# tylerlum/Vine_Robot_IsaacGymEnvs

Measured on AMD Instinct MI355X. Metric: env-steps/sec Vine5LinkMovingBase 16384 envs per GPU, higher is better.
Workload: dtype f32 (env step, rollout inference); update: fp16 GEMM operands and backward-only saved activations (gates, saved cell states, dG, dh), f32 accumulate / recurrent state / heads / loss / optimiser, device-side GradScaler loss scaling (mixed_precision: True = the reference YAML's value, PY:53); rollout

## Files before the change

### vine_robot_isaacgymenvs_amd/csrc/ppo_kernels.hip

```cpp

#include <hip/hip_runtime.h>

#include <cstdio>
#include <cstdlib>

#include "../../include/vine.h"
#include "../../include/vine_ppo.h"
#include "vine_policy_head.h"
#include "vine_ppo_formulas.h"

namespace {

__device__ __forceinline__ float4 ld4(const float* p) { return *reinterpret_cast<const float4*>(p); }
__device__ __forceinline__ void st4(float* p, float4 v) { *reinterpret_cast<float4*>(p) = v; }

typedef unsigned short lp16_t;
typedef __attribute__((__vector_size__(2 * sizeof(float)))) float f32x2_hw;
#ifdef VINE_LP_BF16
typedef __bf16 lp16_hw;
#define VINE_LP16_NAME "bf16"
#define MFMA_LP16_BUILTIN __builtin_amdgcn_mfma_f32_16x16x32_bf16
#define DS_READ_TR16_B64 __builtin_amdgcn_ds_read_tr16_b64_v4bf16
typedef __bf16 lp16_tr_hw;
#define LP16_MAX 3.3895314e38f
#else
typedef _Float16 lp16_hw;
#define VINE_LP16_NAME "fp16"
#define MFMA_LP16_BUILTIN __builtin_amdgcn_mfma_f32_16x16x32_f16
#define DS_READ_TR16_B64 __builtin_amdgcn_ds_read_tr16_b64_v4f16
typedef __fp16 lp16_tr_hw;
#define LP16_MAX 65504.0f
#endif
typedef __attribute__((__vector_size__(2 * sizeof(lp16_hw)))) lp16_hw lp16x2_hw;
__device__ __forceinline__ lp16_t f2lp(float f) {
    const lp16_hw h = (lp16_hw)f;
    return *reinterpret_cast<const lp16_t*>(&h);
}
__device__ __forceinline__ unsigned f2lp2(float lo, float hi) {
    const f32x2_hw v = {lo, hi};
    const lp16x2_hw h = __builtin_convertvector(v, lp16x2_hw);
    return *reinterpret_cast<const unsigned*>(&h);
}
#ifdef VINE_LP_BF16
__device__ __forceinline__ float lp2f(lp16_t h) { return __uint_as_float((unsigned)h << 16); }
__device__ __forceinline__ void unpack2(unsigned r, float& lo, float& hi) {
    lo = __uint_as_float(r << 16);
    hi = __uint_as_float(r & 0xFFFF0000u);
}
#else
__device__ __forceinline__ float lp2f(lp16_t h) { return (float)*reinterpret_cast<const lp16_hw*>(&h); }
__device__ __forceinline__ void unpack2(unsigned r, float& lo, float& hi) {
    const lp16x2_hw h = *reinterpret_cast<const lp16x2_hw*>(&r);
    lo = (float)h[0];
    hi = (float)h[1];
}
#endif
__device__ __forceinline__ float4 ld4(const lp16_t* p) {
    const uint2 r = *reinterpret_cast<const uint2*>(p);
    float4 v;
    unpack2(r.x, v.x, v.y);
    unpack2(r.y, v.z, v.w);
    return v;
}
__device__ __forceinline__ void st4(lp16_t* p, float4 v) {
    uint2 r;
    r.x = f2lp2(v.x, v.y);
    r.y = f2lp2(v.z, v.w);
    *reinterpret_cast<uint2*>(p) = r;
}

template <typename HP>
__global__ void lstm_fwd_kernel(long long B, int H, const float* __restrict__ igates, long long ig_stride,
                                const float* __restrict__ hgates, const float* __restrict__ bias,
                                const float* __restrict__ c_prev, const unsigned char* __restrict__ done,
                                long long done_stride, float* __restrict__ h_out, long long h_stride,
                                float* __restrict__ c_out, HP* __restrict__ gates_act,
                                HP* __restrict__ hp_next, const unsigned char* __restrict__ done_next,
                                long long done_next_stride, long long hp_stride) {
    const int H4 = H >> 2;
    const long long total = B * H4;
    for (long long idx = (long long)blockIdx.x * blockDim.x + threadIdx.x; idx < total;
         idx += (long long)gridDim.x * blockDim.x) {
        const long long b = idx / H4;
        const int j = (int)(idx - b * H4) << 2;
        const float keep = done ? 1.0f - (float)done[b * done_stride] : 1.0f;
        const float* ig = igates + b * ig_stride;
        float4 g[4];
// ... 2060 lines not shown
#pragma unroll
            for (int c = 0; c < 8; ++c)
#pragma unroll
                for (int e = 0; e < 4; ++e) wbits |= (((q[c] >> (8 * e)) & 0xffu) ? 1u : 0u) << (4 * c + e);
            dwords[it] = wbits;
        }
    }
#define WGW_LOAD(S, it)                                                                                        \
    {                                                                                                          \
        const long long t_ = (it) < stages ? (it) : stages - 1;           \
        ra_##S = *reinterpret_cast<const uint4*>(asrc + t_ * 32 * ldy);                                        \
        rb0_##S = *reinterpret_cast<const uint4*>(bsrc0 + t_ * bstep0);                                        \
        rb1_##S = *reinterpret_cast<const uint4*>(bsrc1 + t_ * bstep1);                                        \
        rb2_##S = *reinterpret_cast<const uint4*>(bsrc2 + t_ * bstep2);                                        \
        __builtin_amdgcn_sched_barrier(0);             \
    }
     \
#define WGW_MASKED(v, bit)                                                                                     \
    ([&] { const unsigned m_ = (dw_##bit) ? 0u : 0xffffffffu; return make_uint4((v).x & m_, (v).y & m_, (v).z & m_, (v).w & m_); }())
#define WGW_STORE(S, buf, it)                                                                                  \
    {                                                                                                          \
        const unsigned dw_ = SEQ ? dwords[(it) < stages ? (it) : stages - 1] : 0u;                             \
        const unsigned dw_dbit0 = dw_ & dbit0, dw_dbit1 = dw_ & dbit1, dw_dbit2 = dw_ & dbit2;                 \
        if (aval) *reinterpret_cast<uint4*>(&al[buf][aoff]) = ra_##S;                                          \
        *reinterpret_cast<uint4*>(&bl[buf][boff0]) = WGW_MASKED(rb0_##S, dbit0);                               \
        *reinterpret_cast<uint4*>(&bl[buf][boff1]) = WGW_MASKED(rb1_##S, dbit1);                               \
        if (bval2) *reinterpret_cast<uint4*>(&bl[buf][boff2]) = WGW_MASKED(rb2_##S, dbit2);                    \
    }
    f32x4_t acc[MT][NT];
#pragma unroll
    for (int mt = 0; mt < MT; ++mt)
#pragma unroll
        for (int nt = 0; nt < NT; ++nt) acc[mt][nt] = f32x4_t{0.0f, 0.0f, 0.0f, 0.0f};
    const int g = lane >> 4, il = lane & 15;
    const int ra = (4 * g + (il >> 2)) * PA + 4 * (il & 3) + wm * MT * 16;
    const int rb = (4 * g + (il >> 2)) * PB + 4 * (il & 3) + wn * NT * 16;
#define WGW_COMPUTE(buf)                                                                                       \
    {                                                                                                          \
        const lp16_t* ab = al[buf];                                                                            \
        const lp16_t* bb = bl[buf];                                                                            \
        lp16x8_t af[MT], bfr[NT];                                                                              \
        _Pragma("unroll") for (int mt = 0; mt < MT; ++mt) af[mt] = tr_read8(ab + ra + 16 * mt, 16 * PA);       \
                                                    \
        _Pragma("unroll") for (int nt = 0; nt < NT; ++nt) bfr[nt] = tr_read8(bb + rb + 16 * nt, 16 * PB);      \
        __builtin_amdgcn_sched_barrier(0);                                                                     \
        _Pragma("unroll") for (int nt = 0; nt < NT; ++nt) {                                                    \
            _Pragma("unroll") for (int mt = 0; mt < MT; ++mt)                                                  \
                acc[mt][nt] = MFMA_LP16(af[mt], bfr[nt], acc[mt][nt]);                                         \
        }                                                                                                      \
    }
    WGW_LOAD(e, 0)
    WGW_LOAD(o, 1)
    if (SEQ) __syncthreads();
    WGW_STORE(e, 0, 0)
    __syncthreads();
#pragma unroll 1
    for (int it = 0; it < stages; it += 2) {
        WGW_LOAD(e, it + 2)
        WGW_COMPUTE(0)
        WGW_STORE(o, 1, it + 1)
        __syncthreads();
        WGW_LOAD(o, it + 3)
        WGW_COMPUTE(1)
        WGW_STORE(e, 0, it + 2)
        __syncthreads();
    }
#undef WGW_LOAD
#undef WGW_STORE
#undef WGW_MASKED
#undef WGW_COMPUTE
    const long long mrow = (long long)slice * M + m0 + wm * MT * 16 + 4 * g;
#pragma unroll
    for (int nt = 0; nt < NT; ++nt) {
        const int tg = wn * NT + nt;
        float* base;
        int Nv, col;
        if (tg < NT1) { Nv = Nv1; col = 16 * tg + il; base = part1; }
        else { Nv = Nv2; col = 16 * (tg - NT1) + il; base = part2; }
        if (col < Nv) {
#pragma unroll
            for (int mt = 0; mt < MT; ++mt)
#pragma unroll
                for (int r = 0; r < 4; ++r) base[(mrow + 16 * mt + r) * Nv + col] = acc[mt][nt][r];
        }
    }
}

__device__ __forceinline__ float wave_sum(float v) {
    const int x = dpp_f2i(v);
    float s = v + dpp_i2f(__builtin_amdgcn_update_dpp(0, x, 0x111, 0xf, 0xf, true));
    s += dpp_i2f(__builtin_amdgcn_update_dpp(0, x, 0x112, 0xf, 0xf, true));
    s += dpp_i2f(__builtin_amdgcn_update_dpp(0, x, 0x113, 0xf, 0xf, true));
    s += dpp_i2f(__builtin_amdgcn_update_dpp(0, dpp_f2i(s), 0x114, 0xf, 0xe, true));
    s += dpp_i2f(__builtin_amdgcn_update_dpp(0, dpp_f2i(s), 0x118, 0xf, 0xc, true));
    s += dpp_i2f(__builtin_amdgcn_update_dpp(0, dpp_f2i(s), 0x142, 0xa, 0xf, true));
    s += dpp_i2f(__builtin_amdgcn_update_dpp(0, dpp_f2i(s), 0x143, 0xc, 0xf, true));
    return dpp_i2f(__builtin_amdgcn_readlane(dpp_f2i(s), 63));
}

template <int NV>
__global__ __launch_bounds__(256) void layernorm_fwd_kernel(long long n, const float* __restrict__ x,
                                                            const float* __restrict__ gamma,
                                                            const float* __restrict__ beta, float eps,
                                                            float* __restrict__ y, float* __restrict__ mean_out,
                                                            float* __restrict__ rstd_out) {
    constexpr int H = 256 * NV;
    const int lane = threadIdx.x & 63, wave = threadIdx.x >> 6;
    float4 gm[NV], bt[NV];
#pragma unroll
    for (int v = 0; v < NV; ++v) { gm[v] = ld4(gamma + 256 * v + 4 * lane); bt[v] = ld4(beta + 256 * v + 4 * lane); }
    for (long long r = (long long)blockIdx.x * 4 + wave; r < n; r += (long long)gridDim.x * 4) {
        float4 xv[NV];
        float s = 0.0f;
#pragma unroll
        for (int v = 0; v < NV; ++v) {
            xv[v] = ld4(x + r * H + 256 * v + 4 * lane);
            s += (xv[v].x + xv[v].y) + (xv[v].z + xv[v].w);
        }
        const float mean = wave_sum(s) * (1.0f / H);
        float q = 0.0f;
#pragma unroll
        for (int v = 0; v < NV; ++v) {
            const float a = xv[v].x - mean, b = xv[v].y - mean, c = xv[v].z - mean, d = xv[v].w - mean;
            q += (a * a + b * b) + (c * c + d * d);
        }
        const float rstd = layernorm_rstd(wave_sum(q), H, eps);
#pragma unroll
        for (int v = 0; v < NV; ++v)
            st4(y + r * H + 256 * v + 4 * lane,
                make_float4(layernorm_affine(xv[v].x - mean, rstd, gm[v].x, bt[v].x), layernorm_affine(xv[v].y - mean, rstd, gm[v].y, bt[v].y),
                            layernorm_affine(xv[v].z - mean, rstd, gm[v].z, bt[v].z), layernorm_affine(xv[v].w - mean, rstd, gm[v].w, bt[v].w)));
        if (lane == 0 && mean_out) { mean_out[r] = mean; rstd_out[r] = rstd; }
    }
}

template <int NV>
__global__ __launch_bounds__(256) void layernorm_bwd_kernel(long long n, const float* __restrict__ dy,
                                                            const float* __restrict__ x,
                                                            const float* __restrict__ mean_in,
                                                            const float* __restrict__ rstd_in,
                                                            const float* __restrict__ gamma, float* __restrict__ dx,
                                                            float* __restrict__ partial) {
    constexpr int H = 256 * NV;
    const int lane = threadIdx.x & 63, wave = threadIdx.x >> 6;
    float4 gm[NV];
    float dgm[NV][4], dbt[NV][4];
#pragma unroll
    for (int v = 0; v < NV; ++v) {
        gm[v] = ld4(gamma + 256 * v + 4 * lane);
#pragma unroll
        for (int u = 0; u < 4; ++u) { dgm[v][u] = 0.0f; dbt[v][u] = 0.0f; }
    }
    for (long long r = (long long)blockIdx.x * 4 + wave; r < n; r += (long long)gridDim.x * 4) {
        const float mean = mean_in[r], rstd = rstd_in[r];
        float xh[NV][4], g[NV][4];
        float s1 = 0.0f, s2 = 0.0f;
#pragma unroll
        for (int v = 0; v < NV; ++v) {
            const float4 xv = ld4(x + r * H + 256 * v + 4 * lane), dv = ld4(dy + r * H + 256 * v + 4 * lane);
            const float xa[4] = {xv.x, xv.y, xv.z, xv.w}, da[4] = {dv.x, dv.y, dv.z, dv.w};
            const float ga[4] = {gm[v].x, gm[v].y, gm[v].z, gm[v].w};
#pragma unroll
            for (int u = 0; u < 4; ++u) {
                xh[v][u] = (xa[u] - mean) * rstd;
                g[v][u] = da[u] * ga[u];
                s1 += g[v][u];
// ... 2856 lines not shown
    if (B <= 0 || H <= 0 || (H & 3) || (g_stride & 3) || (dg_stride & 3) || !g_out || !gates_act || !c_new || !c_prev ||
        !dgates || !dc_prev)
        return VINE_ERR_INVALID_ARG;
    const int threads = 256;
    if (bias_partial && (H > 1024 || threads % (int)(H / 4) != 0)) return VINE_ERR_UNSUPPORTED;
    const int blocks = bias_partial ? VINE_PPO_PARTIAL_BLOCKS : grid_for(B * (H / 4), threads);
    if (dgates_bf16)
        hipLaunchKernelGGL(lstm_bwd_kernel<lp16_t>, dim3(blocks), dim3(threads), 0, (hipStream_t)stream, (long long)B,
                           (int)H, g_out, (long long)g_stride, g_rec, dc_next, done_next, (long long)done_next_stride,
                           (const lp16_t*)gates_act, c_new, c_prev, done, (long long)done_stride, (lp16_t*)dgates,
                           (long long)dg_stride,
                           dc_prev, bias_partial, bias_partial_prev);
    else
        hipLaunchKernelGGL(lstm_bwd_kernel<float>, dim3(blocks), dim3(threads), 0, (hipStream_t)stream, (long long)B,
                           (int)H, g_out, (long long)g_stride, g_rec, dc_next, done_next, (long long)done_next_stride,
                           (const float*)gates_act, c_new, c_prev, done, (long long)done_stride, (float*)dgates,
                           (long long)dg_stride,
                           dc_prev, bias_partial, bias_partial_prev);
    return hipGetLastError() == hipSuccess ? VINE_OK : VINE_ERR_DEVICE;
}

int vine_lstm_step_backward_mfma(int64_t B, int64_t H, const float* g_out, int64_t g_stride, const void* dgates_next,
                                 int64_t dgn_stride, const void* w_hh_t, int64_t ldw, const float* dc_next,
                                 const uint8_t* done_next, int64_t done_next_stride, const void* gates_act,
                                 const float* c_new, const float* c_prev, const uint8_t* done, int64_t done_stride,
                                 void* dgates, int64_t dg_stride, float* dc_prev, float* bias_partial,
                                 const float* bias_partial_prev, void* stream) {
    if (B <= 0 || H <= 0 || !g_out || !gates_act || !c_new || !c_prev || !dgates || !dc_prev ||
        (dgates_next != nullptr) != (w_hh_t != nullptr))
        return VINE_ERR_INVALID_ARG;
    if ((B & 63) || (H != 128 && H != 256) || (g_stride & 3) || (dg_stride & 3)) return VINE_ERR_UNSUPPORTED;
    if (dgates_next && ((dgn_stride & 7) || (ldw & 7) || ldw < 4 * H)) return VINE_ERR_INVALID_ARG;
    const dim3 grid((unsigned)(B / 64), (unsigned)(H / 64));
    hipStream_t s = (hipStream_t)stream;
#define VINE_LSTM_BWD_MFMA(NCH)                                                                                        \
    hipLaunchKernelGGL(lstm_bwd_mfma_kernel<NCH>, grid, dim3(256), 0, s, (long long)B, (int)H, g_out,                  \
                       (long long)g_stride, (const lp16_t*)dgates_next, (long long)dgn_stride, (const lp16_t*)w_hh_t,  \
                       (long long)ldw, dc_next, done_next, (long long)done_next_stride, (const lp16_t*)gates_act,      \
                       c_new, c_prev, done, (long long)done_stride, (lp16_t*)dgates, (long long)dg_stride, dc_prev,    \
                       bias_partial, bias_partial_prev)
    if (!dgates_next) VINE_LSTM_BWD_MFMA(0);
    else if (H == 256) VINE_LSTM_BWD_MFMA(8);
    else VINE_LSTM_BWD_MFMA(4);
#undef VINE_LSTM_BWD_MFMA
    return hipGetLastError() == hipSuccess ? VINE_OK : VINE_ERR_DEVICE;
}

int vine_weight_grad_group(int32_t nprob, const int64_t* rows, const int64_t* M, const void* const* dy, const int64_t* ldy,
                           const void* const* x1, const int64_t* ldx1, const int64_t* N1p, const int64_t* Nv1,
                           const void* const* x2, const int64_t* ldx2, const int64_t* N2p, const int64_t* Nv2, const int64_t* NT,
                           const int64_t* slices, float* const* part1, float* const* part2, void* stream) {
    if (nprob <= 0 || nprob > VINE_WGRAD_MAX_PROBLEMS || !rows || !M || !dy || !ldy || !x1 || !ldx1 || !N1p || !Nv1 || !x2 ||
        !ldx2 || !N2p || !Nv2 || !NT || !slices || !part1 || !part2)
        return VINE_ERR_INVALID_ARG;
    WgGroupArgs G;
    int blocks = 0;
    for (int k = 0; k < nprob; ++k) {
        const bool two = N1p[k] > 0;
        if (rows[k] <= 0 || M[k] <= 0 || slices[k] <= 0 || !dy[k] || !x2[k] || !part2[k] || ldy[k] < M[k] || ldx2[k] < N2p[k] ||
            (ldy[k] & 7) || (ldx2[k] & 7) || ((uintptr_t)dy[k] & 15) || ((uintptr_t)x2[k] & 15) || N2p[k] <= 0 || Nv2[k] <= 0 ||
            Nv2[k] > N2p[k] || N1p[k] < 0 ||
            (two && (!x1[k] || !part1[k] || ldx1[k] < N1p[k] || (ldx1[k] & 7) || ((uintptr_t)x1[k] & 15) || Nv1[k] <= 0 ||
                     Nv1[k] > N1p[k])))
            return VINE_ERR_INVALID_ARG;
        if ((NT[k] != 11 && NT[k] != 8 && NT[k] != 2) || (M[k] & 63) || (N1p[k] & 15) || ((N1p[k] + N2p[k]) % (16 * NT[k])) ||
            (slices[k] & 7) || rows[k] % (slices[k] * 32) || slices[k] > 8192)
            return VINE_ERR_UNSUPPORTED;
        WgProblem& P = G.p[k];
        P.dy = (const lp16_t*)dy[k]; P.ldy = ldy[k];
        P.x2 = (const lp16_t*)x2[k]; P.ldx2 = ldx2[k]; P.part2 = part2[k]; P.Nv2 = (int)Nv2[k];
        P.x1 = two ? (const lp16_t*)x1[k] : P.x2; P.ldx1 = two ? ldx1[k] : ldx2[k];
        P.part1 = two ? part1[k] : part2[k]; P.Nv1 = two ? (int)Nv1[k] : (int)Nv2[k];
        P.N1p = (int)N1p[k]; P.M = (int)M[k]; P.NT = (int)NT[k]; P.slices = (int)slices[k];
        P.mtiles = (int)(M[k] / 64); P.ntiles = (int)((N1p[k] + N2p[k]) / (16 * NT[k]));
        P.stages = (int)(rows[k] / slices[k] / 32);
        P.first_block = blocks;
        blocks += P.mtiles * P.ntiles * P.slices;
    }
    G.n = nprob;
    hipLaunchKernelGGL(wgrad_group_kernel, dim3((unsigned)blocks), dim3(256), 0, (hipStream_t)stream, G);
    return hipGetLastError() == hipSuccess ? VINE_OK : VINE_ERR_DEVICE;
}

static int wgrad_cat_wide_launch(int64_t rows, int64_t M, const void* dy, int64_t ldy, const void* x1, int64_t ldx1,
                                 int64_t Nv1, const void* x2, int64_t ldx2, int64_t Nv2, int64_t slices,
                                 float* part1, float* part2, const uint8_t* done, int64_t T, void* stream) {
    const int bm = 128;
    if ((M % bm) || (slices & 7) || rows % (slices * 64) || slices > 8192) return VINE_ERR_UNSUPPORTED;
    const int mtiles = (int)(M / bm), stages = (int)(rows / slices / 32);
    const size_t lds = (size_t)2 * 32 * ((bm + 16) + (352 + 16)) * sizeof(lp16_t);
    if (!ensure_dyn_lds((const void*)wgrad_cat_wide_kernel<6, 2>, lds)) return VINE_ERR_DEVICE;
    hipLaunchKernelGGL((wgrad_cat_wide_kernel<6, 2>), dim3((unsigned)(mtiles * slices)), dim3(512), lds, (hipStream_t)stream,
                       stages, mtiles, (int)slices, (const lp16_t*)dy, (long long)ldy, (const lp16_t*)x1, (long long)ldx1,
                       (const lp16_t*)x2, (long long)ldx2, part1, (int)Nv1, part2, (int)Nv2, (int)M, done,
                       done ? (int)T : (1 << 30));
    return hipGetLastError() == hipSuccess ? VINE_OK : VINE_ERR_DEVICE;
}

int vine_weight_grad_cat_seq_mfma(int64_t rows, int64_t M, const void* dy, int64_t ldy, const void* x1, int64_t ldx1,
                                  int64_t Nv1, const void* h_all, int64_t ldh, const uint8_t* done, int64_t T, int64_t Nv2,
                                  int64_t NT, int64_t slices, float* part1, float* part2, void* stream) {
    if (rows <= 0 || M <= 0 || slices <= 0 || T <= 0 || !dy || !x1 || !h_all || !done || !part1 || !part2 || ldy < M ||
        ldx1 < 96 || ldh < 256 || ((ldy | ldx1 | ldh) & 7) || (((uintptr_t)dy | (uintptr_t)x1 | (uintptr_t)h_all) & 15) ||
        Nv1 <= 0 || Nv1 > 96 || Nv2 <= 0 || Nv2 > 256 || rows % T)
        return VINE_ERR_INVALID_ARG;
    if (NT != 22 || (32 % T) || ((uintptr_t)done & 15) || rows / slices / 32 > 1024) return VINE_ERR_UNSUPPORTED;
    return wgrad_cat_wide_launch(rows, M, dy, ldy, x1, ldx1, Nv1, h_all, ldh, Nv2, slices, part1, part2, done, T, stream);
}

int vine_weight_grad_cat_mfma(int64_t rows, int64_t M, const void* dy, int64_t ldy, const void* x1, int64_t ldx1, int64_t N1p,
                              int64_t Nv1, const void* x2, int64_t ldx2, int64_t N2p, int64_t Nv2, int64_t NT, int64_t slices,
                              float* part1, float* part2, void* stream) {
    if (rows <= 0 || M <= 0 || slices <= 0 || !dy || !x2 || !part2 || ldy < M || ldx2 < N2p || (ldy & 7) || (ldx2 & 7) ||
        ((uintptr_t)dy & 15) || ((uintptr_t)x2 & 15) || N2p <= 0 || Nv2 <= 0 || Nv2 > N2p || N1p < 0 ||
        (N1p > 0 && (!x1 || !part1 || ldx1 < N1p || (ldx1 & 7) || ((uintptr_t)x1 & 15) || Nv1 <= 0 || Nv1 > N1p)))
        return VINE_ERR_INVALID_ARG;
    if (NT == 22) {
        if (N1p != 96 || N2p != 256) return VINE_ERR_UNSUPPORTED;
        return wgrad_cat_wide_launch(rows, M, dy, ldy, x1, ldx1, Nv1, x2, ldx2, Nv2, slices, part1, part2, nullptr, 1, stream);
    }
    if ((NT != 11 && NT != 8 && NT != 2) || (M & 63) || (N1p & 15) || ((N1p + N2p) % (16 * NT)) || (slices & 7) ||
        rows % (slices * 32) || slices > 8192)
        return VINE_ERR_UNSUPPORTED;
    const void* dys[1] = {dy};
    const void* x1s[1] = {x1};
    const void* x2s[1] = {x2};
    float* p1s[1] = {part1};
    float* p2s[1] = {part2};
    return vine_weight_grad_group(1, &rows, &M, dys, &ldy, x1s, &ldx1, &N1p, &Nv1, x2s, &ldx2, &N2p, &Nv2, &NT, &slices, p1s, p2s,
                                  stream);
}

int vine_layernorm_forward(int64_t n, int64_t H, const float* x, const float* gamma, const float* beta, float eps,
                           float* y, float* mean, float* rstd, void* stream) {
    if (n <= 0 || !x || !gamma || !beta || !y || ((mean == nullptr) != (rstd == nullptr))) return VINE_ERR_INVALID_ARG;
    if (H != 256 && H != 512 && H != 1024) return VINE_ERR_UNSUPPORTED;
    const int blocks = (int)((n + 3) / 4 < 256 * 8 ? (n + 3) / 4 : 256 * 8);
    hipStream_t s = (hipStream_t)stream;
    if (H == 256) hipLaunchKernelGGL(layernorm_fwd_kernel<1>, dim3(blocks), dim3(256), 0, s, (long long)n, x, gamma, beta, eps, y, mean, rstd);
    else if (H == 512) hipLaunchKernelGGL(layernorm_fwd_kernel<2>, dim3(blocks), dim3(256), 0, s, (long long)n, x, gamma, beta, eps, y, mean, rstd);
    else hipLaunchKernelGGL(layernorm_fwd_kernel<4>, dim3(blocks), dim3(256), 0, s, (long long)n, x, gamma, beta, eps, y, mean, rstd);
    return hipGetLastError() == hipSuccess ? VINE_OK : VINE_ERR_DEVICE;
}

int vine_layernorm_backward(int64_t n, int64_t H, const float* dy, const float* x, const float* mean, const float* rstd,
                            const float* gamma, float* dx, float* partial, void* stream) {
    if (n <= 0 || !dy || !x || !mean || !rstd || !gamma || !dx || !partial) return VINE_ERR_INVALID_ARG;
    if (H != 256 && H != 512 && H != 1024) return VINE_ERR_UNSUPPORTED;
    const int blocks = VINE_PPO_PARTIAL_BLOCKS;
    hipStream_t s = (hipStream_t)stream;
    if (H == 256) hipLaunchKernelGGL(layernorm_bwd_kernel<1>, dim3(blocks), dim3(256), 0, s, (long long)n, dy, x, mean, rstd, gamma, dx, partial);
    else if (H == 512) hipLaunchKernelGGL(layernorm_bwd_kernel<2>, dim3(blocks), dim3(256), 0, s, (long long)n, dy, x, mean, rstd, gamma, dx, partial);
    else hipLaunchKernelGGL(layernorm_bwd_kernel<4>, dim3(blocks), dim3(256), 0, s, (long long)n, dy, x, mean, rstd, gamma, dx, partial);
    return hipGetLastError() == hipSuccess ? VINE_OK : VINE_ERR_DEVICE;
}

int vine_layernorm_heads_forward(int64_t n, int64_t H, int64_t NH, const float* x, const float* gamma, const float* beta,
                                 float eps, const float* w, const float* wb, float* heads, float* mean, float* rstd,
                                 void* stream) {
    if (n <= 0 || !x || !gamma || !beta || !w || !wb || !heads || !mean || !rstd) return VINE_ERR_INVALID_ARG;
    if (H != 256 || NH < 2 || NH > 5) return VINE_ERR_UNSUPPORTED;
    const int blocks = (int)((n + 3) / 4 < 256 * 8 ? (n + 3) / 4 : 256 * 8);
    hipStream_t s = (hipStream_t)stream;
#define VINE_LNH_FWD(K) hipLaunchKernelGGL(ln_heads_fwd_kernel<K>, dim3(blocks), dim3(256), 0, s, (long long)n, x, gamma, beta, eps, w, wb, heads, mean, rstd)
    if (NH == 2) VINE_LNH_FWD(2); else if (NH == 3) VINE_LNH_FWD(3); else if (NH == 4) VINE_LNH_FWD(4); else VINE_LNH_FWD(5);
#undef VINE_LNH_FWD
    return hipGetLastError() == hipSuccess ? VINE_OK : VINE_ERR_DEVICE;
}

int vine_layernorm_heads_backward(int64_t n, int64_t H, int64_t NH, const float* g, const float* x, const float* mean,
                                  const float* rstd, const float* gamma, const float* beta, const float* w, float* dx,
// ... 690 lines not shown
```

### vine_robot_isaacgymenvs_amd/learning/fused.py

```python
import ctypes as C
import math
import os
from types import SimpleNamespace

import torch
import torch.nn.functional as F


_runtime_ready = set()


def _lib():
    from .. import native
    lib = native.load()
    if torch.cuda.is_available():
        dev = torch.cuda.current_device()
        if dev not in _runtime_ready:
            _runtime_ready.add(dev)
            lib.vine_ppo_runtime_init()
    return lib


def _stream(t):
    if t.device.index != torch.cuda.current_device():
        raise RuntimeError("fused op on %s while the current device is cuda:%d: call torch.cuda.set_device first "
                           "(A2CAgent and train.launch do)" % (t.device, torch.cuda.current_device()))
    return torch.cuda.current_stream(t.device).cuda_stream


def _check(rc, what):
    if rc != 0:
        raise RuntimeError("%s failed with status %d" % (what, rc))


_LP16 = (torch.float16, torch.bfloat16)
_lp = None


def lp_dtype():
    global _lp
    if _lp is None:
        try:
            _lp = torch.float16 if _lib().vine_lp16_format() == b"fp16" else torch.bfloat16
        except (RuntimeError, OSError):
            return torch.float16
    return _lp


def _amp_ptrs(amp):
    if amp is None:
        return None, None
    return amp[0].data_ptr(), amp[1].data_ptr()


def _mm(a, b):
    if a.dtype in _LP16:
        return torch.mm(a, b, out_dtype=torch.float32)
    return a.mm(b)


SPLITK_ROWS = 1024
WGRAD_CAT_WGS = 512
WGRAD_GROUP_WGS = int(os.environ.get("VINE_WGRAD_GROUP_WGS", "256"))
WGRAD_CAT_WIDE = os.environ.get("VINE_WGRAD_CAT_WIDE", "1") != "0"
ROLLOUT_F32_SPLIT = int(os.environ.get("VINE_ROLLOUT_F32_SPLIT", "6"))
ROLLOUT_F32_NSPLIT = os.environ.get("VINE_LSTM_STEP_NSPLIT", "auto")
ROLLOUT_F32_DUAL = os.environ.get("VINE_ROLLOUT_F32_DUAL", os.environ.get("VINE_LSTM_STEP_DUAL", "1")) != "0"
MLP3_F32_SPLIT = os.environ.get("VINE_MLP3_F32_SPLIT", "1") != "0"
MLP3_F32_SPLIT_RT = int(os.environ.get("VINE_MLP3_F32_SPLIT_RT", "0"))
MLP3_PREP = os.environ.get("VINE_MLP3_PREP", "1") != "0"
COPY_SCATTER = os.environ.get("VINE_COPY_SCATTER", "1") != "0"
RIDES = [0]
MLP_PHASE = os.environ.get("VINE_MLP_PHASE", "1") != "0"
BWD_PHASES = os.environ.get("VINE_BWD_PHASES", "1") != "0"
TRUNK_PHASES = os.environ.get("VINE_TRUNK_PHASES", "1") != "0"
PHASE_LAUNCHES = [0]
H_ONCE = os.environ.get("VINE_H_ONCE", "1") != "0"


def rollout_f32_nsplit(rows):
    if ROLLOUT_F32_NSPLIT == "0":
        return 0
    if ROLLOUT_F32_DUAL:
        return 3
    return 1 if (ROLLOUT_F32_NSPLIT == "1" or rows < 16384) else 0


def _carray(ctype, values):
    return (ctype * len(values))(*values)


def _splitk_slices(K):
    s = 1
    while K % (s * 2) == 0 and K // (s * 2) >= SPLITK_ROWS and s < 64:
        s *= 2
    return s


def splitk_tn(dy, x, out=None, batch=None):
    K = dy.shape[0]
    s = _splitk_slices(K)
    if s == 1 or not dy.is_cuda:
        if batch is not None:
            batch.bypassed = True
        if dy.dtype in _LP16:
            r = torch.mm(dy.t(), x, out_dtype=torch.float32)
            return out.copy_(r) if out is not None else r
        return torch.mm(dy.t(), x, out=out) if out is not None else dy.t().mm(x)
    a, b = dy.unflatten(0, (s, K // s)).transpose(1, 2), x.unflatten(0, (s, K // s))
    if dy.dtype not in (torch.float32,) + _LP16 or dy.dtype != x.dtype:
        raise TypeError("splitk_tn: operands must both be fp32 or both 16-bit (got %s, %s)" % (dy.dtype, x.dtype))
    part = torch.bmm(a, b, out_dtype=torch.float32) if dy.dtype in _LP16 else torch.bmm(a, b)
    return column_sums(part, out if out is not None else torch.empty(part.shape[1:], device=part.device), batch=batch)


def _splitk_parts(dy, x):
    K = dy.shape[0]
    s = _splitk_slices(K)
    if s == 1 or not dy.is_cuda:
        return 1, dy.t().mm(x)
    return s, torch.bmm(dy.unflatten(0, (s, K // s)).transpose(1, 2), x.unflatten(0, (s, K // s)))


def weight_grad(dy, x, out=None, batch=None):
    if dy.dtype == lp_dtype() and x.dtype == lp_dtype() and dy.is_cuda:
        o = out if out is not None else torch.empty((dy.shape[1], x.shape[1]), device=dy.device, dtype=torch.float32)
        if o.is_contiguous() and weight_grad_cat(dy, None, x, None, o, batch=batch):
            return o
    return splitk_tn(dy, x, out=out, batch=batch)


def _cat_operand(x, n):
    if not (x.is_cuda and x.dtype == lp_dtype() and x.dim() == 2 and x.shape[0] == n and x.stride(1) == 1
            and x.stride(0) % 8 == 0 and x.data_ptr() % 16 == 0):
        return None
    N = x.shape[1]
    Np = (N + 15) // 16 * 16
    if Np != N and (x.storage_offset() % x.stride(0)) + Np > x.stride(0):
        return None
    return Np, N


def _wgrad_cat_plan(dy, x1, x2, out1, out2, allow_wide=True, wgs=None):
    if not (dy.is_cuda and dy.dtype == lp_dtype() and dy.dim() == 2 and dy.stride(1) == 1
            and dy.stride(0) % 8 == 0 and dy.data_ptr() % 16 == 0 and out2.is_contiguous()
            and (out1 is None or out1.is_contiguous())):
        return None
    n, M = dy.shape
    o2 = _cat_operand(x2, n)
    o1 = _cat_operand(x1, n) if x1 is not None else (0, 0)
    if o1 is None or o2 is None or M % 64:
        return None
    Nt = o1[0] + o2[0]
    NT = 11 if Nt % 176 == 0 else (8 if Nt % 128 == 0 else (2 if Nt == 32 else 0))
    if not NT:
        return None
    wide = allow_wide and WGRAD_CAT_WIDE and o1[0] == 96 and o2[0] == 256 and M % 128 == 0
    if wide:
        NT, tiles, target = 22, M // 128, 256
    else:
        tiles, target = (M // 64) * (Nt // (16 * NT)), (wgs or WGRAD_CAT_WGS)
    S = 8
    while tiles * S < target and n % (128 * S) == 0 and n // (64 * S) >= 8:
        S *= 2
    if n % (64 * S if wide else 32 * S):
        return None
    return n, M, o1[0], o1[1], o2[0], o2[1], NT, S


def h_once_ok(T):
    return H_ONCE and T >= 1 and 32 % T == 0


def masked_previous_hidden(h_all, dones, T):
    H = h_all.shape[1]
    B = h_all.shape[0] // (T + 1)
    prev = h_all.view(B, T + 1, H)[:, :T].reshape(B * T, H)
    if dones is None or dones.numel() == 0:
        return prev.contiguous()
    return (prev * (1 - dones.view(B * T, 1).to(prev.dtype))).contiguous()


def weight_grad_cat(dy, x1, x2, out1, out2, batch=None, seq=None):
    plan = _wgrad_cat_plan(dy, x1, x2 if seq is None else x2[:dy.shape[0]], out1, out2)
    if plan is None:
        return False
    n, M, N1p, Nv1, N2p, Nv2, NT, S = plan
    if seq is not None and (NT != 22 or x1 is None or not h_once_ok(seq[1]) or seq[0].data_ptr() % 16
                            or n // S // 32 > 1024 or x2.shape[0] != n // seq[1] * (seq[1] + 1) or not x2.is_contiguous()):
        return False
    part2 = torch.empty((S, M, Nv2), device=dy.device, dtype=torch.float32)
    part1 = torch.empty((S, M, Nv1), device=dy.device, dtype=torch.float32) if x1 is not None else None
    if seq is not None:
        dones, T = seq
        assert dones.numel() == n and dones.dtype == torch.uint8
        _check(_lib().vine_weight_grad_cat_seq_mfma(n, M, dy.data_ptr(), dy.stride(0), x1.data_ptr(), x1.stride(0), Nv1,
                                                    x2.data_ptr(), x2.stride(0), dones.data_ptr(), T, Nv2, NT, S,
                                                    part1.data_ptr(), part2.data_ptr(), _stream(dy)),
               "vine_weight_grad_cat_seq_mfma")
    else:
        _check(_lib().vine_weight_grad_cat_mfma(n, M, dy.data_ptr(), dy.stride(0), x1.data_ptr() if x1 is not None else None,
                                                x1.stride(0) if x1 is not None else 0, N1p, Nv1, x2.data_ptr(), x2.stride(0),
                                                N2p, Nv2, NT, S, part1.data_ptr() if part1 is not None else None,
                                                part2.data_ptr(), _stream(dy)), "vine_weight_grad_cat_mfma")
    if part1 is not None:
        column_sums(part1, out1, batch=batch)
    column_sums(part2, out2, batch=batch)
    return True


class WeightGradGroup:
    MAX = 6

    def __init__(self):
        self.jobs = []

    def add(self, dy, x, out, batch):
        if len(self.jobs) >= self.MAX or batch is None:
            return False
        plan = _wgrad_cat_plan(dy, None, x, None, out, allow_wide=False, wgs=WGRAD_GROUP_WGS)
        if plan is None:
            return False
        n, M, _n1p, _nv1, N2p, Nv2, NT, S = plan
        part = torch.empty((S, M, Nv2), device=dy.device, dtype=torch.float32)
        self.jobs.append((n, M, dy, x, N2p, Nv2, NT, S, part))
        column_sums(part, out, batch=batch)
        return True

    def flush(self):
        if not self.jobs:
            return
        k = len(self.jobs)
        i64 = lambda f: _carray(C.c_int64, [f(j) for j in self.jobs])
        ptr = lambda f: _carray(C.c_void_p, [f(j) for j in self.jobs])
        zeros, nulls = _carray(C.c_int64, [0] * k), _carray(C.c_void_p, [None] * k)
        _check(_lib().vine_weight_grad_group(
            k, i64(lambda j: j[0]), i64(lambda j: j[1]), ptr(lambda j: j[2].data_ptr()), i64(lambda j: j[2].stride(0)),
            nulls, zeros, zeros, zeros, ptr(lambda j: j[3].data_ptr()), i64(lambda j: j[3].stride(0)), i64(lambda j: j[4]),
            i64(lambda j: j[5]), i64(lambda j: j[6]), i64(lambda j: j[7]), nulls, ptr(lambda j: j[8].data_ptr()),
            _stream(self.jobs[0][2])), "vine_weight_grad_group")
        self.jobs = []

# ... 1091 lines not shown
```

Baseline: 28.04 million.

## Split wide concatenated wgrad into paired N-halves with intra-block K split

Adds a wgrad_cat_pair_kernel that splits the 352-wide [x1|x2] output into two 176-column tiles per M tile. Each block splits the K dimension across two wave groups, stages 64 rows per step, and reduces the two partial accumulators through LDS at the end. Doubling the tile count lowers the per-block accumulator footprint and raises parallelism. The Python planner also counts twice as many tiles when choosing slices. The cost is reloading the dy operand for each N-half plus an extra LDS reduction, and the old path stays reachable through VINE_WGRAD_CAT_WIDE=352.

```diff
diff --git a/vine_robot_isaacgymenvs_amd/csrc/ppo_kernels.hip b/vine_robot_isaacgymenvs_amd/csrc/ppo_kernels.hip
--- a/vine_robot_isaacgymenvs_amd/csrc/ppo_kernels.hip
+++ b/vine_robot_isaacgymenvs_amd/csrc/ppo_kernels.hip
@@ -3,6 +3,7 @@
 
 #include <cstdio>
 #include <cstdlib>
+#include <cstring>
 
 #include "../../include/vine.h"
 #include "../../include/vine_ppo.h"
@@ -2229,6 +2230,171 @@
             for (int mt = 0; mt < MT; ++mt)
 #pragma unroll
                 for (int r = 0; r < 4; ++r) base[(mrow + 16 * mt + r) * Nv + col] = acc[mt][nt][r];
+        }
+    }
+}
+
+template <int NT1>
+__global__ __launch_bounds__(512) void wgrad_cat_pair_kernel(int stages, int mtiles, int slices, const lp16_t* __restrict__ dy,
+                                                             long long ldy, const lp16_t* __restrict__ x1, long long ldx1,
+                                                             const lp16_t* __restrict__ x2, long long ldx2,
+                                                             float* __restrict__ part1, int Nv1, float* __restrict__ part2,
+                                                             int Nv2, int M, const unsigned char* __restrict__ done, int T) {
+    constexpr int NT = 11, MT = 2, WM = 4, WK = 2, TH = 64 * WM * WK;
+    constexpr int BM = 16 * MT * WM, BN = 16 * NT, N1 = 16 * NT1;
+    constexpr int PA = BM + 16, PB = BN;
+    constexpr int APC = BM / 8, AP = 32 * APC;
+    constexpr int BC = BN / 8, BP = 32 * WK * BC;
+    const bool SEQ = done != nullptr;
+    static_assert(AP == TH && BP <= 3 * TH && BP > 2 * TH && BP % 64 == 0 && N1 % 8 == 0 && N1 < BN,
+                  "staging slots: one piece of dy per thread and half, 3 of [x1 | x2] per thread");
+    static_assert(((PA * 2) % 64) == 32 && ((PB * 2) % 64) == 32, "pitches: odd multiples of 32 B");
+    extern __shared__ __attribute__((aligned(16))) unsigned char wg_lds[];
+    lp16_t (*al)[32 * WK * PA] = reinterpret_cast<lp16_t (*)[32 * WK * PA]>(wg_lds);
+    lp16_t (*bl)[32 * WK * PB] = reinterpret_cast<lp16_t (*)[32 * WK * PB]>(wg_lds + 2 * 32 * WK * PA * sizeof(lp16_t));
+    const int tid = threadIdx.x, lane = tid & 63;
+    const int wave = __builtin_amdgcn_readfirstlane(tid >> 6);
+    const int wm = wave & 3, wk = wave >> 2;
+    const int xcd = blockIdx.x & 7, q = blockIdx.x >> 3, tps = 2 * mtiles;
+    const int slice = xcd * (slices >> 3) + q / tps, tile = q % tps;
+    const int m0 = (tile >> 1) * BM, n0 = (tile & 1) * BN;
+    const long long R = 32LL * stages;
+    const long long k0 = (long long)slice * 2 * R;
+    const lp16_t* asrc0 = dy + (k0 + tid / APC) * ldy + m0 + 8 * (tid % APC);
+    const lp16_t* asrc1 = asrc0 + R * ldy;
+    const int aoff = (tid / APC) * PA + 8 * (tid % APC);
+#define WGP_SRC(i)                                                                                             \
+    const lp16_t* bsrc##i; long long bstep##i; int boff##i; bool bval##i, dhalf##i;                            \
+    unsigned dbit##i = 0;                          \
+    {                                                                                                          \
+        const int p = tid + TH * (i);                                                                          \
+        bval##i = p < BP;                                                                                      \
+        const int pp = bval##i ? p : 0, r = pp / BC, c = n0 + 8 * (pp % BC);                                   \
+        const long long k = k0 + (r >> 5) * R + (r & 31);                                                      \
+        dhalf##i = r >= 32;                                                                                    \
+        if (c < N1) {                                                                                          \
+            bsrc##i = x1 + k * ldx1 + c; bstep##i = 32 * ldx1;                                                 \
+        } else {                                                                                               \
+                                                \
+            if (SEQ && bval##i) dbit##i = 1u << (r & 31);                                                      \
+            bsrc##i = x2 + (k + k / T) * ldx2 + (c - N1); bstep##i = (32 + 32 / T) * ldx2;                     \
+        }                                                                                                      \
+        boff##i = r * PB + 8 * (pp % BC);                                                                      \
+    }
+    WGP_SRC(0) WGP_SRC(1) WGP_SRC(2)
+#undef WGP_SRC
+    uint4 ra0_e, ra1_e, rb0_e, rb1_e, rb2_e, ra0_o, ra1_o, rb0_o, rb1_o, rb2_o;
+    __shared__ unsigned dwords[1024];
+    if (SEQ) {
+        for (int w = tid; w < 2 * stages; w += TH) {
+            const uint4 a = *reinterpret_cast<const uint4*>(done + k0 + 32 * w);
+            const uint4 b = *reinterpret_cast<const uint4*>(done + k0 + 32 * w + 16);
+            const unsigned q8[8] = {a.x, a.y, a.z, a.w, b.x, b.y, b.z, b.w};
+            unsigned wbits = 0;
+#pragma unroll
+            for (int c = 0; c < 8; ++c)
+#pragma unroll
+                for (int e = 0; e < 4; ++e) wbits |= (((q8[c] >> (8 * e)) & 0xffu) ? 1u : 0u) << (4 * c + e);
+            dwords[w] = wbits;
+        }
+    }
+#define WGP_LOAD(S, it)                                                                                        \
+    {                                                                                                          \
+        const long long t_ = (it) < stages ? (it) : stages - 1;           \
+        ra0_##S = *reinterpret_cast<const uint4*>(asrc0 + t_ * 32 * ldy);                                      \
+        ra1_##S = *reinterpret_cast<const uint4*>(asrc1 + t_ * 32 * ldy);                                      \
+        rb0_##S = *reinterpret_cast<const uint4*>(bsrc0 + t_ * bstep0);                                        \
+        rb1_##S = *reinterpret_cast<const uint4*>(bsrc1 + t_ * bstep1);                                        \
+        rb2_##S = *reinterpret_cast<const uint4*>(bsrc2 + t_ * bstep2);                                        \
+        __builtin_amdgcn_sched_barrier(0);             \
+    }
+     \
+#define WGP_MASKED(v, bit)                                                                                     \
+    ([&] { const unsigned m_ = (dw_##bit) ? 0u : 0xffffffffu; return make_uint4((v).x & m_, (v).y & m_, (v).z & m_, (v).w & m_); }())
+#define WGP_STORE(S, buf, it)                                                                                  \
+    {                                                                                                          \
+        const int w_ = (it) < stages ? (it) : stages - 1;                                                      \
+        const unsigned dw0_ = SEQ ? dwords[w_] : 0u, dw1_ = SEQ ? dwords[stages + w_] : 0u;                    \
+        const unsigned dw_dbit0 = (dhalf0 ? dw1_ : dw0_) & dbit0, dw_dbit1 = (dhalf1 ? dw1_ : dw0_) & dbit1,   \
+                       dw_dbit2 = (dhalf2 ? dw1_ : dw0_) & dbit2;                                              \
+        *reinterpret_cast<uint4*>(&al[buf][aoff]) = ra0_##S;                                                   \
+        *reinterpret_cast<uint4*>(&al[buf][aoff + 32 * PA]) = ra1_##S;                                         \
+        *reinterpret_cast<uint4*>(&bl[buf][boff0]) = WGP_MASKED(rb0_##S, dbit0);                               \
+        *reinterpret_cast<uint4*>(&bl[buf][boff1]) = WGP_MASKED(rb1_##S, dbit1);                               \
+        if (bval2) *reinterpret_cast<uint4*>(&bl[buf][boff2]) = WGP_MASKED(rb2_##S, dbit2);                    \
+    }
+    f32x4_t acc[MT][NT];
+#pragma unroll
+    for (int mt = 0; mt < MT; ++mt)
+#pragma unroll
+        for (int nt = 0; nt < NT; ++nt) acc[mt][nt] = f32x4_t{0.0f, 0.0f, 0.0f, 0.0f};
+    const int g = lane >> 4, il = lane & 15;
+    const int ra = (32 * wk + 4 * g + (il >> 2)) * PA + 4 * (il & 3) + wm * MT * 16;
+    const int rb = (32 * wk + 4 * g + (il >> 2)) * PB + 4 * (il & 3);
+#define WGP_COMPUTE(buf)                                                                                       \
+    {                                                                                                          \
+        const lp16_t* ab = al[buf];                                                                            \
+        const lp16_t* bb = bl[buf];                                                                            \
+        lp16x8_t af[MT], bfr[NT];                                                                              \
+        _Pragma("unroll") for (int mt = 0; mt < MT; ++mt) af[mt] = tr_read8(ab + ra + 16 * mt, 16 * PA);       \
+              \
+        _Pragma("unroll") for (int nt = 0; nt < NT; ++nt) bfr[nt] = tr_read8(bb + rb + 16 * nt, 16 * PB);      \
+        __builtin_amdgcn_sched_barrier(0);                                                                     \
+        _Pragma("unroll") for (int nt = 0; nt < NT; ++nt) {                                                    \
+            _Pragma("unroll") for (int mt = 0; mt < MT; ++mt)                                                  \
+                acc[mt][nt] = MFMA_LP16(af[mt], bfr[nt], acc[mt][nt]);                                         \
+        }                                                                                                      \
+    }
+    WGP_LOAD(e, 0)
+    WGP_LOAD(o, 1)
+    if (SEQ) __syncthreads();
+    WGP_STORE(e, 0, 0)
+    __syncthreads();
+#pragma unroll 1
+    for (int it = 0; it < stages; it += 2) {
+        WGP_LOAD(e, it + 2)
+        WGP_COMPUTE(0)
+        WGP_STORE(o, 1, it + 1)
+        __syncthreads();
+        WGP_LOAD(o, it + 3)
+        WGP_COMPUTE(1)
+        WGP_STORE(e, 0, it + 2)
+        __syncthreads();
+    }
+#undef WGP_LOAD
+#undef WGP_STORE
+#undef WGP_MASKED
+#undef WGP_COMPUTE
+    static_assert((size_t)WM * WK * NT * 64 * sizeof(f32x4_t) <= 90112, "hand-over area (host: dynamic LDS)");
+    f32x4_t* xl = reinterpret_cast<f32x4_t*>(wg_lds);
+    f32x4_t* xs = xl + wave * NT * 64 + lane;
+    const f32x4_t* xr = xl + (wave ^ 4) * NT * 64 + lane;
+    if (wk == 0) {
+#pragma unroll
+        for (int nt = 0; nt < NT; ++nt) xs[64 * nt] = acc[1][nt];
+    } else {
+#pragma unroll
+        for (int nt = 0; nt < NT; ++nt) xs[64 * nt] = acc[0][nt];
+    }
+    __syncthreads();
+    if (wk == 0) {
+#pragma unroll
+        for (int nt = 0; nt < NT; ++nt) acc[0][nt] = acc[0][nt] + xr[64 * nt];
+    } else {
+#pragma unroll
+        for (int nt = 0; nt < NT; ++nt) acc[0][nt] = xr[64 * nt] + acc[1][nt];
+    }
+    const long long mrow = (long long)slice * M + m0 + wm * MT * 16 + 16 * wk + 4 * g;
+#pragma unroll
+    for (int nt = 0; nt < NT; ++nt) {
+        const int vc = n0 + 16 * nt;
+        float* base;
+        int Nv, col;
+        if (vc < N1) { Nv = Nv1; col = vc + il; base = part1; }
+        else { Nv = Nv2; col = vc - N1 + il; base = part2; }
+        if (col < Nv) {
+#pragma unroll
+            for (int r = 0; r < 4; ++r) base[(mrow + r) * Nv + col] = acc[0][nt][r];
         }
     }
 }
@@ -5251,11 +5417,27 @@
     return hipGetLastError() == hipSuccess ? VINE_OK : VINE_ERR_DEVICE;
 }
 
+static bool wgrad_cat_force_352() {
+    const char* e = getenv("VINE_WGRAD_CAT_WIDE");
+    return e && !strcmp(e, "352");
+}
+
 static int wgrad_cat_wide_launch(int64_t rows, int64_t M, const void* dy, int64_t ldy, const void* x1, int64_t ldx1,
                                  int64_t Nv1, const void* x2, int64_t ldx2, int64_t Nv2, int64_t slices,
                                  float* part1, float* part2, const uint8_t* done, int64_t T, void* stream) {
     const int bm = 128;
     if ((M % bm) || (slices & 7) || rows % (slices * 64) || slices > 8192) return VINE_ERR_UNSUPPORTED;
+    if (rows % (slices * 128) == 0 && !wgrad_cat_force_352()) {
+        const int mtiles = (int)(M / bm), stages = (int)(rows / slices / 64);
+        const size_t stage_lds = (size_t)2 * 64 * ((bm + 16) + 176) * sizeof(lp16_t), pair_lds = 90112;
+        const size_t lds = stage_lds > pair_lds ? stage_lds : pair_lds;
+        if (!ensure_dyn_lds((const void*)wgrad_cat_pair_kernel<6>, lds)) return VINE_ERR_DEVICE;
+        hipLaunchKernelGGL((wgrad_cat_pair_kernel<6>), dim3((unsigned)(mtiles * 2 * slices)), dim3(512), lds,
+                           (hipStream_t)stream, stages, mtiles, (int)slices, (const lp16_t*)dy, (long long)ldy,
+                           (const lp16_t*)x1, (long long)ldx1, (const lp16_t*)x2, (long long)ldx2, part1, (int)Nv1, part2,
+                           (int)Nv2, (int)M, done, done ? (int)T : (1 << 30));
+        return hipGetLastError() == hipSuccess ? VINE_OK : VINE_ERR_DEVICE;
+    }
     const int mtiles = (int)(M / bm), stages = (int)(rows / slices / 32);
     const size_t lds = (size_t)2 * 32 * ((bm + 16) + (352 + 16)) * sizeof(lp16_t);
     if (!ensure_dyn_lds((const void*)wgrad_cat_wide_kernel<6, 2>, lds)) return VINE_ERR_DEVICE;
diff --git a/vine_robot_isaacgymenvs_amd/learning/fused.py b/vine_robot_isaacgymenvs_amd/learning/fused.py
--- a/vine_robot_isaacgymenvs_amd/learning/fused.py
+++ b/vine_robot_isaacgymenvs_amd/learning/fused.py
@@ -63,6 +63,7 @@
 WGRAD_CAT_WGS = 512
 WGRAD_GROUP_WGS = int(os.environ.get("VINE_WGRAD_GROUP_WGS", "256"))
 WGRAD_CAT_WIDE = os.environ.get("VINE_WGRAD_CAT_WIDE", "1") != "0"
+WGRAD_CAT_PAIR = os.environ.get("VINE_WGRAD_CAT_WIDE", "1") != "352"
 ROLLOUT_F32_SPLIT = int(os.environ.get("VINE_ROLLOUT_F32_SPLIT", "6"))
 ROLLOUT_F32_NSPLIT = os.environ.get("VINE_LSTM_STEP_NSPLIT", "auto")
 ROLLOUT_F32_DUAL = os.environ.get("VINE_ROLLOUT_F32_DUAL", os.environ.get("VINE_LSTM_STEP_DUAL", "1")) != "0"
@@ -157,7 +158,7 @@
         return None
     wide = allow_wide and WGRAD_CAT_WIDE and o1[0] == 96 and o2[0] == 256 and M % 128 == 0
     if wide:
-        NT, tiles, target = 22, M // 128, 256
+        NT, tiles, target = 22, M // 128 * (2 if WGRAD_CAT_PAIR else 1), 256
     else:
         tiles, target = (M // 64) * (Nt // (16 * NT)), (wgs or WGRAD_CAT_WGS)
     S = 8
```

After: 28.31 million, median of 6. About the same (+1.0%).
